# CDCgov/NowcastAutoGP

Measured on AMD Instinct MI355X. Metric: particle-logml/s (fit+forecast hot path: covariance assembly + Cholesky + logml + predictive per (particle, scenario) item), n=2048 64-particle SMC, higher is better.
Workload: dtype f64

## Files before the change

### nowcastautogp_amd/csrc/ngp_col_kernels.h

```cpp
#pragma once
#include <algorithm>

#include "ngp_mfma.h"

namespace ngp {

struct NoProbe {
    __device__ __forceinline__ void mark(int) {}
    template <class T>
    __device__ __forceinline__ void mark_after(int, T) {}
    __device__ __forceinline__ void drain() {}
    __device__ __forceinline__ void emit_diag(int, int, int) {}
    __device__ __forceinline__ void emit_col(int, int, int, int, int, int, bool) {}
    __device__ __forceinline__ void begin(int, int, int) {}
    __device__ __forceinline__ void sweep(int) {}
};

__device__ __forceinline__ void sqrt_and_rcp(double a, double &d, double &r) {
    double y = __builtin_amdgcn_rsq(a);
    const double h = 0.5 * a;
    y = y * fma(-h * y, y, 1.5);
    y = y * fma(-h * y, y, 1.5);
    d = a * y;
    d = fma(fma(-d, d, a), 0.5 * y, d);
    r = fma(fma(-d, y, 1.0), y, y);
}

__device__ __forceinline__ int tri(int r, int c) { return ((r * (r + 1)) >> 1) + c; }
constexpr int TRI = NB * (NB + 1) / 2;

template <class Probe = NoProbe>
__global__ __launch_bounds__(256, 4) void chol_diag_kernel(JobGeom g, ChunkPtrs p, int j, int k0) {
    __shared__ double Mt[TRI];
    __shared__ double Lt[TRI];
    __shared__ double pan[NB][4];
    __shared__ double dblk[16];
    __shared__ double dinvd[4];
    __shared__ double rdg[NB];
    __shared__ double logs[NB];
    __shared__ double Ts[TB][TB + 1];
    __shared__ int bad;
    const int item = blockIdx.x;
    const int tid = threadIdx.x, lane = tid & 63;
    const int wave = __builtin_amdgcn_readfirstlane(tid >> 6);
    const long ld = g.ld;
    double *Lit = p.L + (long)item * g.item_stride;
    double *Lj = Lit + (long)j * NB * ld;
    const int kmax = j * NB;
    const int r16 = lane & 15, q = lane >> 4;
    const int wr = wave >> 1, wc = wave & 1;
    Probe probe;
    probe.mark_after(0, lane);

    if (tid == 0) bad = 0;

    if (!(wr == 0 && wc == 1)) {
        double acc4[2][2][4];
#pragma unroll
        for (int a = 0; a < 2; ++a)
#pragma unroll
            for (int b = 0; b < 2; ++b)
#pragma unroll
                for (int r = 0; r < 4; ++r) acc4[a][b][r] = 0.0;
        const double *pa = Lj + (long)(32 * wr + r16) * ld + 2 * q;
        const double *pb = Lj + (long)(32 * wc + r16) * ld + 2 * q;
        double kt[2][2][4];
#pragma unroll
        for (int mt = 0; mt < 2; ++mt)
#pragma unroll
            for (int nt = 0; nt < 2; ++nt)
#pragma unroll
                for (int s = 0; s < 4; ++s)
                    kt[mt][nt][s] = Lj[(long)(32 * wr + 16 * mt + q + 4 * s) * ld + kmax +
                                       32 * wc + 16 * nt + r16];
        for (int kc = k0; kc < kmax; kc += 16) {
            double a[2][4], b[2][4];
#pragma unroll
            for (int u = 0; u < 2; ++u) {
                const f64x2 alo = *reinterpret_cast<const f64x2 *>(pa + (long)u * 16 * ld + kc);
                const f64x2 ahi = *reinterpret_cast<const f64x2 *>(pa + (long)u * 16 * ld + kc + 8);
                const f64x2 blo = *reinterpret_cast<const f64x2 *>(pb + (long)u * 16 * ld + kc);
                const f64x2 bhi = *reinterpret_cast<const f64x2 *>(pb + (long)u * 16 * ld + kc + 8);
                a[u][0] = alo.x; a[u][1] = alo.y; a[u][2] = ahi.x; a[u][3] = ahi.y;
                b[u][0] = blo.x; b[u][1] = blo.y; b[u][2] = bhi.x; b[u][3] = bhi.y;
            }
#pragma unroll
            for (int s = 0; s < 4; ++s)
#pragma unroll
                for (int nt = 0; nt < 2; ++nt) {
                    const Rot4 br = rot4(b[nt][s]);
#pragma unroll
                    for (int mt = 0; mt < 2; ++mt) mfma16_as_4(acc4[mt][nt], a[mt][s], br);
                }
        }
        f64x4 acc[2][2];
#pragma unroll
        for (int a = 0; a < 2; ++a)
#pragma unroll
            for (int b = 0; b < 2; ++b) acc[a][b] = to_d16(acc4[a][b]);
#pragma unroll
        for (int mt = 0; mt < 2; ++mt)
#pragma unroll
            for (int nt = 0; nt < 2; ++nt)
#pragma unroll
                for (int s = 0; s < 4; ++s) {
                    const int M = 32 * wr + 16 * mt + q + 4 * s, N = 32 * wc + 16 * nt + r16;
                    if (M >= N) Mt[tri(M, N)] = kt[mt][nt][s] - acc[mt][nt][s];
                }
    }
    __syncthreads();
    probe.mark_after(1, lane);

    const int bi = tid >> 4, bj = tid & 15;
    {
        double a[4][4];
#pragma unroll
        for (int r = 0; r < 4; ++r)
#pragma unroll
            for (int c = 0; c < 4; ++c) {
                const int R = 4 * bi + r, C = 4 * bj + c;
                a[r][c] = (R >= C) ? Mt[tri(R, C)] : 0.0;
            }
        for (int kb = 0; kb < NB / 4; ++kb) {
            if (bi == kb && bj == kb) {
                double dks[4];
#pragma unroll
                for (int kc = 0; kc < 4; ++kc) {
                    const double akk = a[kc][kc];
                    double dk, inv;
                    sqrt_and_rcp(akk, dk, inv);
                    if (!(akk > 0.0) && bad == 0) bad = 4 * kb + kc + 1;
                    dks[kc] = dk;
                    dinvd[kc] = inv;
                    rdg[4 * kb + kc] = inv;
#pragma unroll
                    for (int r = 0; r < 4; ++r)
                        if (r > kc) a[r][kc] *= inv;
#pragma unroll
                    for (int c = 0; c < 4; ++c)
                        if (c > kc) {
#pragma unroll
                            for (int r = 0; r < 4; ++r)
                                if (r >= c) a[r][c] -= a[r][kc] * a[c][kc];
                        }
                }
#pragma unroll
                for (int r = 0; r < 4; ++r)
#pragma unroll
                    for (int c = 0; c < 4; ++c) {
                        if (r == c) a[r][c] = dks[r];
                        if (c > r) a[r][c] = 0.0;
                        dblk[4 * r + c] = a[r][c];
                    }
            }
            __syncthreads();
            if (bj == kb && bi > kb) {
#pragma unroll
                for (int c = 0; c < 4; ++c) {
                    const double inv = dinvd[c];
#pragma unroll
                    for (int r = 0; r < 4; ++r) {
                        double v = a[r][c];
#pragma unroll
                        for (int pp = 0; pp < 4; ++pp)
                            if (pp < c) v -= a[r][pp] * dblk[4 * c + pp];
                        a[r][c] = v * inv;
                    }
                }
#pragma unroll
                for (int r = 0; r < 4; ++r)
#pragma unroll
                    for (int c = 0; c < 4; ++c) pan[4 * bi + r][c] = a[r][c];
            }
            __syncthreads();
            if (bj > kb && bi >= bj) {
                double li[4][4], lj[4][4];
#pragma unroll
                for (int r = 0; r < 4; ++r)
#pragma unroll
                    for (int pp = 0; pp < 4; ++pp) {
                        li[r][pp] = pan[4 * bi + r][pp];
                        lj[r][pp] = pan[4 * bj + r][pp];
                    }
#pragma unroll
                for (int pp = 0; pp < 4; ++pp)
#pragma unroll
                    for (int r = 0; r < 4; ++r)
#pragma unroll
                        for (int c = 0; c < 4; ++c) a[r][c] -= li[r][pp] * lj[c][pp];
            }
        }
#pragma unroll
        for (int r = 0; r < 4; ++r) {
            const int R = 4 * bi + r;
            f64x2 lo, hi;
            lo.x = (R >= 4 * bj) ? a[r][0] : 0.0;
            lo.y = (R >= 4 * bj + 1) ? a[r][1] : 0.0;
            hi.x = (R >= 4 * bj + 2) ? a[r][2] : 0.0;
            hi.y = (R >= 4 * bj + 3) ? a[r][3] : 0.0;
            double *dst = Lj + (long)R * ld + kmax + 4 * bj;
            *reinterpret_cast<f64x2 *>(dst) = lo;
            *reinterpret_cast<f64x2 *>(dst + 2) = hi;
#pragma unroll
            for (int c = 0; c < 4; ++c)
                if (R >= 4 * bj + c) Lt[tri(R, 4 * bj + c)] = a[r][c];
        }
    }
    __syncthreads();
    probe.mark_after(2, lane);
    if (tid < NB) logs[tid] = log(Lt[tri(tid, tid)]);

    if (tid < NB) {
        const int b = tid >> 4, c = tid & 15;
        double x[TB];
#pragma unroll
        for (int i = 0; i < TB; ++i) {
            double sum = (i == c) ? 1.0 : 0.0;
            int off = tri(TB * b + i, TB * b);
            if (i > 0) asm volatile("" : "+v"(off) : "v"(x[i - 1]));
            const double *lrow = &Lt[off];
#pragma unroll
            for (int pp = 0; pp < i; ++pp) sum -= lrow[pp] * x[pp];
            x[i] = sum * rdg[TB * b + i];
        }
#pragma unroll
        for (int i = 0; i < TB; ++i)
            if (i >= c) Mt[tri(TB * b + i, TB * b + c)] = x[i];
    }
    __syncthreads();
    probe.mark_after(3, lane);
    {
        const int ra = tid >> 4, cb = tid & 15;
        for (int dist = 1; dist < NB / TB; ++dist)
            for (int ct = dist; ct < NB / TB; ++ct) {
                const int jt = ct - dist;
                double t = 0.0;
                for (int kt = jt; kt < ct; ++kt)
#pragma unroll
                    for (int pp = 0; pp < TB; ++pp) {
                        const double mv = Mt[tri(TB * kt + pp, TB * jt + cb)];
                        t += Lt[tri(TB * ct + ra, TB * kt + pp)] * ((kt > jt || pp >= cb) ? mv : 0.0);
                    }
                Ts[ra][cb] = t;
                __syncthreads();
                double mv = 0.0;
#pragma unroll
                for (int pp = 0; pp < TB; ++pp) {
                    const double md = Mt[tri(TB * ct + ra, TB * ct + pp)];
                    mv -= ((pp <= ra) ? md : 0.0) * Ts[pp][cb];
                }
                Mt[tri(TB * ct + ra, TB * jt + cb)] = mv;
                __syncthreads();
            }
    }
    probe.mark_after(4, lane);
    {
        double *dv = p.dinv + (long)item * (NB * NB);
        for (int e = tid; e < NB * NB; e += 256) {
            const int strip = e >> 6, l = e & 63;
            const int cb4 = strip >> 2, jt = strip & 3;
            const int R = 4 * cb4 + (l & 3), C = 16 * jt + 4 * ((l >> 2) & 3) + (l >> 4);
            dv[e] = (R >= C) ? Mt[tri(R, C)] : 0.0;
        }
    }
    if (tid == 0) {
        double s = 0.0;
        for (int k = 0; k < NB; ++k) s += logs[k];
        p.logdet[item] += s;
        if (bad && p.info[item] == 0) p.info[item] = kmax + bad;
    }
    probe.mark_after(5, lane);
    probe.emit_diag(j, tid, item);
}

template <int NF>
struct Frag8 {
    f64x2 v[NF];
};
template <int NF>
__device__ __forceinline__ void load_frag8(Frag8<NF> &f, const double *p, long ld) {
#pragma unroll
    for (int u = 0; u < NF; ++u) f.v[u] = *reinterpret_cast<const f64x2 *>(p + (long)u * 16 * ld);
}
template <int NA>
__device__ __forceinline__ void mfma_frag8(double (&acc)[NA][4][4], const Frag8<NA> &a,
                                           const Frag8<4> &b) {
#pragma unroll
    for (int it = 0; it < 4; ++it) {
        const Rot4 br = rot4(b.v[it].x);
#pragma unroll
        for (int jt = 0; jt < NA; ++jt) mfma16_as_4(acc[jt][it], a.v[jt].x, br);
    }
#pragma unroll
    for (int it = 0; it < 4; ++it) {
        const Rot4 br = rot4(b.v[it].y);
#pragma unroll
        for (int jt = 0; jt < NA; ++jt) mfma16_as_4(acc[jt][it], a.v[jt].y, br);
    }
}

template <int NA>
__device__ __forceinline__ void gemm_rows(double (&acc)[NA][4][4], const double *pa,
                                          const double *pb, long ld, int k0, int k1) {
    if (k1 <= k0) return;
    Frag8<NA> a0, a1;
    Frag8<4> b0, b1;
    load_frag8(a0, pa + k0, ld);
    load_frag8(b0, pb + k0, ld);
    for (int kc = k0; kc < k1; kc += 16) {
        load_frag8(a1, pa + kc + 8, ld);
        load_frag8(b1, pb + kc + 8, ld);
        mfma_frag8(acc, a0, b0);
        if (kc + 16 < k1) {
            load_frag8(a0, pa + kc + 16, ld);
            load_frag8(b0, pb + kc + 16, ld);
        }
        mfma_frag8(acc, a1, b1);
    }
}

constexpr int EPI_PITCH = 66;
constexpr int EPI_M_BYTES = NB * NB * 8;
constexpr int EPI_WAVE_BYTES = 16 * EPI_PITCH * 8;
constexpr int EPI_LDS_BYTES = EPI_M_BYTES + 4 * EPI_WAVE_BYTES;

__device__ __forceinline__ void stage_mstrips(double *lds_m, const double *mstrips, int tid) {
#pragma unroll
    for (int i = 0; i < 8; ++i) {
        const int idx = tid + 256 * i;
        reinterpret_cast<f64x2 *>(lds_m)[idx] = reinterpret_cast<const f64x2 *>(mstrips)[idx];
    }
}

template <bool SHADOW = false, bool SYNTH = false, class Probe = NoProbe, bool KROWS = false>
__device__ __forceinline__ void solve_and_store_lds(const double (*acc4)[4][4], double *Lr,
                                                    const double *lds_m, long ld, int kmax,
                                                    int lane, double *buf, Probe &probe,
                                                    float *Lr32 = nullptr,
                                                    float *tmax_out = nullptr, int synth = 0,
                                                    const double *ksl = nullptr, int nit = 4) {
    double amax = 0.0;
    const int n16 = lane & 15, isub = lane >> 4;
    const int jj0 = 4 * (n16 >> 2) + isub;
    const double *ksl0 = ksl ? ksl + 15 - jj0 : nullptr;
    f64x2 kvr[8];
    double kvp[4][4];
    const int hrow = lane >> 5, c2 = 2 * (lane & 31);
    bool from_rows = KROWS && ksl0 == nullptr;
    if constexpr (SYNTH) from_rows = from_rows && synth == 0;
    auto k_elems = [&](int it, double (&kv)[4][4]) {
        if (ksl0) {
#pragma unroll
            for (int jt = 0; jt < 4; ++jt)
#pragma unroll
                for (int r = 0; r < 4; ++r)
                    kv[jt][r] = ksl0[((n16 + 4 * r) & 15) + 16 * (it - jt + 3)];
            return;
        }
        if constexpr (SYNTH) {
            if (synth) {
#pragma unroll
                for (int jt = 0; jt < 4; ++jt)
#pragma unroll
                    for (int r = 0; r < 4; ++r) {
                        const int i = 16 * it + ((n16 + 4 * r) & 15);
                        kv[jt][r] = (synth == 2 && i == 16 * jt + jj0) ? 1.0 : 0.0;
                    }
                return;
            }
        }
        if constexpr (!KROWS) {
#pragma unroll
            for (int jt = 0; jt < 4; ++jt)
#pragma unroll
                for (int r = 0; r < 4; ++r) {
                    const int i = 16 * it + ((n16 + 4 * r) & 15);
                    kv[jt][r] = Lr[(long)i * ld + kmax + 16 * jt + jj0];
                }
        }
    };
    auto load_k = [&](int it) {
        if constexpr (KROWS) {
            if (!from_rows) return;
#pragma unroll
            for (int i = 0; i < 8; ++i)
                kvr[i] = *reinterpret_cast<const f64x2 *>(Lr + (long)(16 * it + 2 * i + hrow) * ld + kmax + c2);
        } else {
            k_elems(it, kvp);
        }
    };
    auto take_k = [&](int it, double (&kv)[4][4]) {
        if constexpr (KROWS) {
            if (!from_rows) {
                k_elems(it, kv);
                return;
            }
#pragma unroll
            for (int i = 0; i < 8; ++i)
                *reinterpret_cast<f64x2 *>(buf + (2 * i + hrow) * EPI_PITCH + c2) = kvr[i];
#pragma unroll
            for (int jt = 0; jt < 4; ++jt)
#pragma unroll
                for (int r = 0; r < 4; ++r)
                    kv[jt][r] = buf[((n16 + 4 * r) & 15) * EPI_PITCH + 16 * jt + jj0];
        } else {
#pragma unroll
            for (int jt = 0; jt < 4; ++jt)
#pragma unroll
                for (int r = 0; r < 4; ++r) kv[jt][r] = kvp[jt][r];
        }
    };
    load_k(0);
#pragma unroll
    for (int it = 0; it < 4; ++it) {
        if (it >= nit) break;
        double c4[4][4];
        take_k(it, c4);
#pragma unroll
        for (int jt = 0; jt < 4; ++jt)
#pragma unroll
            for (int r = 0; r < 4; ++r) c4[jt][r] = c4[jt][r] - acc4[jt][it][r];
        probe.mark_after(12 + 3 * it, c4[3][3] + c4[0][0] + c4[1][2] + c4[2][1]);
        if (it + 1 < nit) load_k(it + 1);
        double ms[2][4];
        ms[0][0] = lds_m[lane];
#pragma unroll
        for (int cb4 = 0; cb4 < 16; ++cb4) {
            const int ct = cb4 >> 2;
            if (cb4 + 1 < 16) {
#pragma unroll
                for (int jt = 0; jt <= ((cb4 + 1) >> 2); ++jt)
                    ms[(cb4 + 1) & 1][jt] = lds_m[((cb4 + 1) * 4 + jt) * 64 + lane];
            }
            double R[4] = {0.0, 0.0, 0.0, 0.0};
#pragma unroll
            for (int jt = 0; jt <= ct; ++jt) {
#pragma unroll
                for (int r = 0; r < 4; ++r) R[r] = mfma4(ms[cb4 & 1][jt], c4[jt][r], R[r]);
            }
            double x = R[0];
            x += dpp_f64<ROW_ROR4, 0xF>(R[1], R[1]);
            x += dpp_f64<ROW_ROR8, 0xF>(R[2], R[2]);
            x += dpp_f64<ROW_ROR12, 0xF>(R[3], R[3]);
            buf[n16 * EPI_PITCH + 4 * cb4 + isub] = x;
        }
        probe.mark_after(13 + 3 * it, it);
#pragma unroll
        for (int w = 0; w < 8; ++w) {
            const int idx = w * 64 + lane, row = idx >> 5, cp = idx & 31;
            const f64x2 v = *reinterpret_cast<const f64x2 *>(buf + row * EPI_PITCH + 2 * cp);
            *reinterpret_cast<f64x2 *>(Lr + (long)(16 * it + row) * ld + kmax + 2 * cp) = v;
            if constexpr (SHADOW) {
                typedef float f32x2 __attribute__((ext_vector_type(2)));
                f32x2 vf;
                vf.x = (float)v.x;
                vf.y = (float)v.y;
                *reinterpret_cast<f32x2 *>(Lr32 + (long)(16 * it + row) * ld + kmax + 2 * cp) = vf;
                amax = fmax(amax, fmax(fabs(v.x), fabs(v.y)));
            }
        }
        probe.mark_after(14 + 3 * it, it);
        __builtin_amdgcn_sched_barrier(0);
    }
    if constexpr (SHADOW) {
#pragma unroll
        for (int off = 32; off > 0; off >>= 1) amax = fmax(amax, __shfl_xor(amax, off, 64));
        if (lane == 0) *tmax_out = __double2float_ru(amax);
    }
}

__device__ __forceinline__ void subtract_in_place_perm(double *rows, long ld, int c0,
                                                       const double (*acc4)[4][4], int lane,
                                                       bool fresh = false,
                                                       const double *ksl = nullptr, int nit = 4) {
    const int n16 = lane & 15, isub = lane >> 4;
    const int jj0 = 4 * (n16 >> 2) + isub;
    double *base = rows + c0 + jj0;
    long roff[4];
#pragma unroll
    for (int r = 0; r < 4; ++r) roff[r] = (long)((n16 + 4 * r) & 15) * ld;
    if (ksl) {
        const double *ksl0 = ksl + 15 - jj0;
#pragma unroll
        for (int it = 0; it < 4; ++it)
#pragma unroll
            for (int jt = 0; jt < 4; ++jt)
#pragma unroll
                for (int r = 0; r < 4; ++r)
                    base[(long)(16 * it) * ld + roff[r] + 16 * jt] =
                        ksl0[((n16 + 4 * r) & 15) + 16 * (it - jt + 3)] - acc4[jt][it][r];
        return;
    }
    if (fresh) {
#pragma unroll
        for (int it = 0; it < 4; ++it)
#pragma unroll
            for (int jt = 0; jt < 4; ++jt)
#pragma unroll
                for (int r = 0; r < 4; ++r)
                    base[(long)(16 * it) * ld + roff[r] + 16 * jt] = -acc4[jt][it][r];
        return;
    }
    double v[2][4][4];
#pragma unroll
    for (int jt = 0; jt < 4; ++jt)
#pragma unroll
        for (int r = 0; r < 4; ++r) v[0][jt][r] = base[roff[r] + 16 * jt];
#pragma unroll
    for (int it = 0; it < 4; ++it) {
        if (it >= nit) break;
        if (it + 1 < nit) {
#pragma unroll
            for (int jt = 0; jt < 4; ++jt)
#pragma unroll
                for (int r = 0; r < 4; ++r)
                    v[(it + 1) & 1][jt][r] = base[(long)(16 * (it + 1)) * ld + roff[r] + 16 * jt];
        }
#pragma unroll
        for (int jt = 0; jt < 4; ++jt)
#pragma unroll
            for (int r = 0; r < 4; ++r)
                base[(long)(16 * it) * ld + roff[r] + 16 * jt] = v[it & 1][jt][r] - acc4[jt][it][r];
    }
}

__device__ __forceinline__ void subtract_in_place_rows(double *rows, long ld, int c0,
                                                       const double (*acc4)[4][4], int lane,
                                                       double *tl, bool fresh = false,
                                                       const double *ksl = nullptr, int nit = 4) {
    const int n16 = lane & 15, isub = lane >> 4;
    const int jj0 = 4 * (n16 >> 2) + isub;
    const int hrow = lane >> 5, c2 = 2 * (lane & 31);
    double *base = rows + c0 + c2;
    auto load_rows = [&](int it, f64x2 (&kv)[8]) {
        if (ksl) {
#pragma unroll
            for (int i = 0; i < 8; ++i) {
                const int d = 63 + 16 * it + 2 * i + hrow - c2;
                kv[i].x = ksl[d];
                kv[i].y = ksl[d - 1];
            }
        } else if (fresh) {
#pragma unroll
            for (int i = 0; i < 8; ++i) kv[i].x = kv[i].y = 0.0;
        } else {
#pragma unroll
            for (int i = 0; i < 8; ++i)
                kv[i] = *reinterpret_cast<const f64x2 *>(base + (long)(16 * it + 2 * i + hrow) * ld);
        }
    };
    f64x2 kv[2][8];
    load_rows(0, kv[0]);
#pragma unroll
    for (int it = 0; it < 4; ++it) {
        if (it >= nit) break;
        if (it + 1 < nit) load_rows(it + 1, kv[(it + 1) & 1]);
#pragma unroll
        for (int jt = 0; jt < 4; ++jt)
#pragma unroll
            for (int r = 0; r < 4; ++r)
                tl[((n16 + 4 * r) & 15) * EPI_PITCH + 16 * jt + jj0] = acc4[jt][it][r];
#pragma unroll
        for (int i = 0; i < 8; ++i) {
            const f64x2 a = *reinterpret_cast<const f64x2 *>(tl + (2 * i + hrow) * EPI_PITCH + c2);
            f64x2 o;
            o.x = kv[it & 1][i].x - a.x;
            o.y = kv[it & 1][i].y - a.y;
            *reinterpret_cast<f64x2 *>(base + (long)(16 * it + 2 * i + hrow) * ld) = o;
        }
    }
}

__device__ __forceinline__ void struct_slice(double *ksl, const JobGeom &g, const ChunkPtrs &p,
                                             int item, int row0, int col0, int lane) {
    const double *tab = p.tab + (long)item * g.maxstat * g.R;
    const int d0 = row0 - col0 - 63;
    ksl[lane] = tab[(long)g.toep * (d0 + lane)];
    if (lane < 63) ksl[64 + lane] = tab[(long)g.toep * (d0 + 64 + lane)];
}
constexpr int TOEP_LDS_BYTES = 4 * 128 * 8;

struct ColStep {
    int j;
    int k0;
    int nmain;
    int ntiles;
    int groups;
    int splits;
    int first_touch;
    double c32, jitter;
};
__device__ __forceinline__ long tmax_index(const JobGeom &g, int row_tile, int col) {
    return (long)row_tile * g.nb0 + col;
}

template <bool MIXED, bool IDENT = false, bool TOEP = false>
__global__ __launch_bounds__(256, 2) void chol_col_kernel(JobGeom g, ChunkPtrs p, int Bc,
                                                          ColStep st) {
    __shared__ __attribute__((aligned(16))) char epi[EPI_LDS_BYTES + (TOEP ? TOEP_LDS_BYTES : 0)];
    const int wg = blockIdx.x;
    const int xcd = wg & 7, idx = wg >> 3;
    const int slot = (idx / st.groups) * 8 + xcd;
    const int grp = idx % st.groups;
    if (slot >= Bc) return;
    const int item = p.items ? p.items[slot] : slot;
    const int tid = threadIdx.x, lane = tid & 63;
    const int wave = __builtin_amdgcn_readfirstlane(tid >> 6);
    const int tile = grp * 4 + wave;
    bool valid = tile < st.ntiles;
    int kbeg = st.k0;
    int synth = 0;
    if constexpr (IDENT) {
        if (valid && tile >= st.nmain) {
            const int a = tile - st.nmain;
            if (a < g.nb0) {
                if (a > st.j) valid = false;
                else if (a * NB > kbeg) kbeg = a * NB;
                synth = (a == st.j) ? 2 : 1;
            }
        }
    }

    const int j = st.j;
    const long ld = g.ld;
    double *Lit = p.L + (long)item * g.item_stride;
    const int kmax = j * NB;
    const int r16 = lane & 15, q = lane >> 4;

    double acc4[4][4][4];
#pragma unroll
    for (int a = 0; a < 4; ++a)
#pragma unroll
        for (int b = 0; b < 4; ++b)
#pragma unroll
            for (int r = 0; r < 4; ++r) acc4[a][b][r] = 0.0;

    const int vt = valid ? tile : 0;
    const long rowbase = (vt < st.nmain) ? (long)(j + 1 + vt) * NB
                                         : (long)g.n0 + (long)(vt - st.nmain) * NB;
    double *Lr = Lit + rowbase * ld;
    const double *Lj = Lit + (long)j * NB * ld;
    const double *pa = Lj + (long)r16 * ld + 2 * q;
    const double *pb = Lr + (long)r16 * ld + 2 * q;
    if (valid) gemm_rows<4>(acc4, pa, pb, ld, kbeg, kmax);
    const double *ksl = nullptr;
    if constexpr (TOEP) {
        if (valid && tile < st.nmain && prog_structure(p.progs + item)) {
            double *sl = reinterpret_cast<double *>(epi + EPI_LDS_BYTES) + wave * 128;
            struct_slice(sl, g, p, item, (int)rowbase, kmax, lane);
            ksl = sl;
        }
    }
    stage_mstrips(reinterpret_cast<double *>(epi), p.dinv + (long)item * (NB * NB), tid);
    __syncthreads();
    if (!valid) return;
    NoProbe probe;
    if constexpr (MIXED) {
        const int rt = (tile < st.nmain) ? j + 1 + tile : g.nb0 + (tile - st.nmain);
        solve_and_store_lds<true>(
            acc4, Lr, reinterpret_cast<const double *>(epi), ld, kmax, lane,
            reinterpret_cast<double *>(epi + EPI_M_BYTES + wave * EPI_WAVE_BYTES), probe,
            p.L32 + (long)item * g.item_stride + rowbase * ld,
            p.tmax + (long)item * (g.nb0 + g.naux_pad / NB) * g.nb0 + tmax_index(g, rt, j));
    } else {
        solve_and_store_lds<false, IDENT>(
            acc4, Lr, reinterpret_cast<const double *>(epi), ld, kmax, lane,
            reinterpret_cast<double *>(epi + EPI_M_BYTES + wave * EPI_WAVE_BYTES), probe, nullptr,
            nullptr, synth, ksl);
    }
}

template <bool MIXED, class Probe = NoProbe, bool IDENT = false>
__global__ __launch_bounds__(256, 2) void chol_col_thin_kernel(JobGeom g, ChunkPtrs p, int Bc,
                                                               ColStep st) {
    constexpr int A_BYTES = NB * NB * 8;
    constexpr int TAIL = (4 * EPI_WAVE_BYTES > A_BYTES) ? 4 * EPI_WAVE_BYTES : A_BYTES;
    __shared__ __attribute__((aligned(1024))) char smem[EPI_M_BYTES + TAIL];
    typedef __attribute__((address_space(3))) void *lds_ptr;
    const int wg = blockIdx.x;
    const int xcd = wg & 7, idx = wg >> 3;
    const int slot = (idx / st.groups) * 8 + xcd;
    const int grp = idx % st.groups;
    if (slot >= Bc) return;
    const int item = p.items ? p.items[slot] : slot;
    const int tid = threadIdx.x, lane = tid & 63;
    const int wave = __builtin_amdgcn_readfirstlane(tid >> 6);
    const int tile = grp * 4 + wave;
    bool valid = tile < st.ntiles;
    const int j = st.j;
    const int kmax = j * NB, k0 = kmax - NB;
    bool update = true;
    int synth = 0;
    if constexpr (IDENT) {
        if (valid && tile >= st.nmain) {
            const int a = tile - st.nmain;
            if (a < g.nb0) {
                if (a > j) valid = false;
                else if (a * NB > k0) update = false;
                if (a == j) synth = 2;
            }
        }
    }
    const long ld = g.ld;
    double *Lit = p.L + (long)item * g.item_stride;
    const int r16 = lane & 15, q = lane >> 4;
    Probe probe;
    probe.mark_after(0, lane);

    {
        const __amdgpu_buffer_rsrc_t rl = __builtin_amdgcn_make_buffer_rsrc(
            Lit, 0, (int)(g.item_stride * (long)sizeof(double)), 0x00020000);
        const __amdgpu_buffer_rsrc_t rm = __builtin_amdgcn_make_buffer_rsrc(
            p.dinv + (long)item * (NB * NB), 0, NB * NB * 8, 0x00020000);
        const int rbit = lane >> 5, sl = lane & 31;
#pragma unroll
        for (int i = 0; i < 8; ++i) {
            const int key = (2 * i + rbit) & 7;
            const unsigned voff = (unsigned)((rbit * ld + 2 * (sl ^ key)) * 8);
            const unsigned soff = (unsigned)__builtin_amdgcn_readfirstlane(
                (int)((((long)kmax + 2 * (8 * wave + i)) * ld + k0) * 8));
            lds_ptr dst = (lds_ptr)(smem + EPI_M_BYTES + (8 * wave + i) * 1024);
            __builtin_amdgcn_raw_ptr_buffer_load_lds(rl, dst, 16, voff, soff, 0, 0);
        }
#pragma unroll
        for (int i = 0; i < 8; ++i) {
            lds_ptr dst = (lds_ptr)(smem + (8 * wave + i) * 1024);
            __builtin_amdgcn_raw_ptr_buffer_load_lds(rm, dst, 16, (unsigned)(lane * 16),
                                                     (unsigned)((8 * wave + i) * 1024), 0, 0);
        }
    }

    double acc4[4][4][4];
#pragma unroll
    for (int a = 0; a < 4; ++a)
#pragma unroll
        for (int b = 0; b < 4; ++b)
#pragma unroll
            for (int r = 0; r < 4; ++r) acc4[a][b][r] = 0.0;

    const int vt = valid ? tile : 0;
    const long rowbase = (vt < st.nmain) ? (long)(j + 1 + vt) * NB
                                         : (long)g.n0 + (long)(vt - st.nmain) * NB;
    double *Lr = Lit + rowbase * ld;
    const double *pb = Lr + (long)r16 * ld + k0 + 2 * q;
    const bool mult = valid && update;
    Frag8<4> b[4];
    if (mult) {
#pragma unroll
        for (int sg = 0; sg < 4; ++sg) load_frag8(b[sg], pb + 8 * sg, ld);
    }
    __syncthreads();
    probe.mark_after(1, lane);
    if (mult) {
        const char *Ab = smem + EPI_M_BYTES + r16 * 512;
        const int key = r16 & 7;
#pragma unroll
        for (int sg = 0; sg < 8; ++sg) {
            Frag8<4> a;
#pragma unroll
            for (int u = 0; u < 4; ++u)
                a.v[u] = *reinterpret_cast<const f64x2 *>(Ab + u * (16 * 512) +
                                                          (((4 * sg + q) ^ key) << 4));
            mfma_frag8(acc4, a, b[sg & 3]);
            if (sg + 4 < 8) load_frag8(b[sg & 3], pb + 8 * (sg + 4), ld);
        }
    }
    probe.mark_after(2, acc4[0][0][0] + acc4[3][3][3]);
    __syncthreads();
    probe.mark_after(3, lane);
    probe.mark_after(4, lane);
    if (!valid) return;
    double *buf = reinterpret_cast<double *>(smem + EPI_M_BYTES + wave * EPI_WAVE_BYTES);
    if constexpr (MIXED) {
        const int rt = (tile < st.nmain) ? j + 1 + tile : g.nb0 + (tile - st.nmain);
        solve_and_store_lds<true, false, Probe, true>(
            acc4, Lr, reinterpret_cast<const double *>(smem), ld, kmax, lane, buf, probe,
            p.L32 + (long)item * g.item_stride + rowbase * ld,
            p.tmax + (long)item * (g.nb0 + g.naux_pad / NB) * g.nb0 + tmax_index(g, rt, j));
    } else {
        int nit = (tile >= st.nmain && g.naux - NB * (tile - st.nmain) <= 16) ? 1 : 4;
        if (IDENT && tile < st.nmain && g.n_real - NB * (j + 1 + tile) <= 16) nit = 1;
        solve_and_store_lds<false, IDENT, Probe, true>(acc4, Lr, reinterpret_cast<const double *>(smem), ld,
                                          kmax, lane, buf, probe, nullptr, nullptr, synth, nullptr,
                                          nit);
    }
    probe.mark_after(5, lane);
    probe.drain();
    probe.mark_after(6, lane);
    probe.emit_col(j, lane, wg, wave, item, tile, true);
}

constexpr int LDS_KC = 16;

typedef float f32x4 __attribute__((ext_vector_type(4)));
typedef float f32x16 __attribute__((ext_vector_type(16)));


template <bool MIXED, class Probe = NoProbe, bool IDENT = false, int SPLITK = 0>
__global__ __launch_bounds__(256, 2) void chol_col_glds_kernel(JobGeom g, ChunkPtrs p, int Bc,
                                                               ColStep st) {
    constexpr int ROWB = 128, BLKB = 8 * ROWB + 128, STAGE = 32 * BLKB;
    auto row_off = [](int row) { return (row >> 3) * BLKB + (row & 7) * ROWB; };
    __shared__ __attribute__((aligned(1024))) char smem[2 * STAGE];
    typedef __attribute__((address_space(3))) void *lds_ptr;

    const int wg = blockIdx.x;
    const int xcd = wg & 7, idx = wg >> 3;
    const int per_item = SPLITK == 1 ? st.groups * st.splits : st.groups;
    const int slot = (idx / per_item) * 8 + xcd;
    const int grp = SPLITK == 1 ? (idx % per_item) / st.splits : idx % st.groups;
    const int piece = SPLITK == 1 ? (idx % per_item) % st.splits : 0;
    if (slot >= Bc) return;
    const int item = (MIXED && p.order) ? p.order[slot] : slot;
    const int tid = threadIdx.x, lane = tid & 63;
    const int wave = __builtin_amdgcn_readfirstlane(tid >> 6);
    const int ltile = wave >> 1, col = wave & 1;
    const int tile0 = grp * 2;
    const int tile = tile0 + ltile;
    bool valid = tile < st.ntiles;

    const int j = st.j;
    Probe probe;
    probe.mark(0);
    const long ld = g.ld;
    double *Lit = p.L + (long)item * g.item_stride;
    const int kmax = j * NB;
    bool structured = false;
    if constexpr (!MIXED && !IDENT) {
        if (g.toep && st.first_touch && valid && tile < st.nmain && !(col && tile == 0))
            structured = prog_structure(p.progs + item) != 0;
    }
    int kbeg = st.k0;
    int synth = 0;
    if constexpr (IDENT) {
        const int a = tile - st.nmain;
        if (tile < st.ntiles && a >= 0 && a < g.nb0) synth = (a == j) ? 2 : 1;
    }
    if (IDENT && tile0 >= st.nmain) {
        int kfirst = kmax + 1;
#pragma unroll
        for (int u = 0; u < 2; ++u) {
            const int a = tile0 + u - st.nmain;
            if (tile0 + u >= st.ntiles) continue;
            const int ks = (a >= g.nb0) ? st.k0 : (a > j) ? kmax + 1 : max(st.k0, a * NB);
            kfirst = min(kfirst, ks);
        }
        if (kfirst > kmax) return;
        kbeg = kfirst;
        const int a = tile - st.nmain;
        if (valid && a < g.nb0 && a > j) valid = false;
    }
    int nit = 4;
    if constexpr (!MIXED && SPLITK == 0) {
        if (IDENT && !valid) nit = 0;
        else if (valid && tile >= st.nmain && g.naux - NB * (tile - st.nmain) <= 16) nit = 1;
        else if (IDENT && valid && tile < st.nmain && g.n_real - NB * (j + 1 + tile) <= 16) nit = 1;
    }
    const int r16 = lane & 15, q = lane >> 4;
    auto tile_row0 = [&](int t) -> long {
        if (t >= st.ntiles) t = st.ntiles - 1;
        return (t < st.nmain) ? (long)(j + 1 + t) * NB : (long)g.n0 + (long)(t - st.nmain) * NB;
    };
    const __amdgpu_buffer_rsrc_t rsrc = __builtin_amdgcn_make_buffer_rsrc(
        Lit, 0, (int)(g.item_stride * (long)sizeof(double)), 0x00020000);
    long src_row0;
    if (wave < 2) src_row0 = (long)j * NB + 64 * wave;
    else src_row0 = tile_row0(tile0 + (wave - 2));
    const unsigned soff_base = (unsigned)__builtin_amdgcn_readfirstlane((int)(src_row0 * ld * 8));
    const unsigned row_step8 = (unsigned)(8 * ld * 8);
    const unsigned voff_even = (unsigned)(((lane >> 3) * ld + 2 * ((lane & 7) ^ ((lane >> 4) & 7))) * 8);
    const unsigned voff_odd = (unsigned)(((lane >> 3) * ld + 2 * ((lane & 7) ^ ((4 + (lane >> 4)) & 7))) * 8);
    auto stage = [&](int buf, int k) {
        const unsigned kb = (unsigned)k * 8u;
#pragma unroll
        for (int i = 0; i < 8; ++i) {
            lds_ptr dst = (lds_ptr)(smem + buf * STAGE + (8 * wave + i) * BLKB);
            __builtin_amdgcn_raw_ptr_buffer_load_lds(rsrc, dst, 16, (i & 1) ? voff_odd : voff_even,
                                                     soff_base + i * row_step8 + kb, 0, 0);
        }
    };
    unsigned a_addr[4], b_addr[4][4];
    {
        const int arow = 64 * col + r16;
        const int akey = (r16 >> 1) & 7;
#pragma unroll
        for (int s = 0; s < 4; ++s)
            a_addr[s] = (unsigned)(row_off(arow) + (((2 * s + (q >> 1)) ^ akey) << 4) + (q & 1) * 8);
#pragma unroll
        for (int r = 0; r < 4; ++r) {
            const int rr = (r16 + 4 * r) & 15;
            const int brow = 128 + 64 * ltile + rr;
            const int bkey = (rr >> 1) & 7;
#pragma unroll
            for (int s = 0; s < 4; ++s)
                b_addr[r][s] =
                    (unsigned)(row_off(brow) + (((2 * s + (q >> 1)) ^ bkey) << 4) + (q & 1) * 8);
        }
    }

    double acc4[4][4][4];
#pragma unroll
    for (int a = 0; a < 4; ++a)
#pragma unroll
        for (int b = 0; b < 4; ++b)
#pragma unroll
            for (int r = 0; r < 4; ++r) acc4[a][b][r] = 0.0;

    auto mult64 = [&](const char *buf, auto nit_c) {
        constexpr int NIT = decltype(nit_c)::value;
#pragma unroll
        for (int s = 0; s < 4; ++s) {
            double a[4];
#pragma unroll
            for (int u = 0; u < 4; ++u)
                a[u] = *reinterpret_cast<const double *>(buf + a_addr[s] + u * 2 * BLKB);
#pragma unroll
            for (int it = 0; it < NIT; ++it) {
                Rot4 br;
                br.r0 = *reinterpret_cast<const double *>(buf + b_addr[0][s] + it * 2 * BLKB);
                br.r1 = *reinterpret_cast<const double *>(buf + b_addr[1][s] + it * 2 * BLKB);
                br.r2 = *reinterpret_cast<const double *>(buf + b_addr[2][s] + it * 2 * BLKB);
                br.r3 = *reinterpret_cast<const double *>(buf + b_addr[3][s] + it * 2 * BLKB);
#pragma unroll
                for (int jt = 0; jt < 4; ++jt) mfma16_as_4(acc4[jt][it], a[jt], br);
            }
        }
    };

    if constexpr (SPLITK == 2) {
    } else if constexpr (!MIXED) {
        int nchunks = (kmax - kbeg) / LDS_KC;
        if constexpr (SPLITK == 1) {
            const int per = (nchunks + st.splits - 1) / st.splits;
            const int c0 = min(piece * per, nchunks);
            nchunks = min(c0 + per, nchunks) - c0;
            kbeg += c0 * LDS_KC;
        }
        if (nchunks > 0) {
            stage(0, kbeg);
            __syncthreads();
            if (IDENT && nit == 0) {
                for (int c = 0; c < nchunks; ++c) {
                    if (c + 1 < nchunks) stage((c & 1) ^ 1, kbeg + (c + 1) * LDS_KC);
                    __syncthreads();
                }
            } else if (nit == 1) {
                for (int c = 0; c < nchunks; ++c) {
                    const int cur = c & 1;
                    if (c + 1 < nchunks) stage(cur ^ 1, kbeg + (c + 1) * LDS_KC);
                    mult64(smem + cur * STAGE, std::integral_constant<int, 1>{});
                    __syncthreads();
                }
            } else {
                for (int c = 0; c < nchunks; ++c) {
                    const int cur = c & 1;
                    if (c + 1 < nchunks) stage(cur ^ 1, kbeg + (c + 1) * LDS_KC);
                    mult_chunk_pipelined<2 * BLKB>(acc4, smem + cur * STAGE, a_addr, b_addr);
                    __syncthreads();
                    if (c == 0) probe.mark(1);
                    if (c == nchunks / 2) probe.mark(2);
                }
            }
        }
    } else {
        const int nkt = j;
        const int nbt = g.nb0 + g.naux_pad / NB;
        const float *tm = p.tmax + (long)item * nbt * g.nb0;
        const int t1 = min(tile0 + 1, st.ntiles - 1);
        const int rt0 = (tile0 < st.nmain) ? j + 1 + tile0 : g.nb0 + (tile0 - st.nmain);
        const int rt1 = (t1 < st.nmain) ? j + 1 + t1 : g.nb0 + (t1 - st.nmain);
        const double lim = st.c32 * (p.progs[item].noise + st.jitter);
        unsigned long long m32lo, m32hi;
        {
            bool c[2];
#pragma unroll
            for (int h = 0; h < 2; ++h) {
                const int kt = lane + 64 * h;
                c[h] = false;
                if (kt < nkt) {
                    const float ta = fmaxf(tm[tmax_index(g, j, kt)], tm[tmax_index(g, j + 1, kt)]);
                    const float tb = fmaxf(tm[tmax_index(g, rt0, kt)], tm[tmax_index(g, rt1, kt)]);
                    c[h] = (double)ta * (double)tb <= lim;
                }
            }
            m32lo = __ballot(c[0]);
            m32hi = __ballot(c[1]);
        }
        const unsigned long long inlo = nkt >= 64 ? ~0ull : ((1ull << nkt) - 1ull);
        const unsigned long long inhi = nkt <= 64 ? 0ull : (nkt >= 128 ? ~0ull : ((1ull << (nkt - 64)) - 1ull));
        unsigned long long m64lo = inlo & ~m32lo, m64hi = inhi & ~m32hi;
        const int n32 = __popcll(m32lo) + __popcll(m32hi);
        const int n64 = __popcll(m64lo) + __popcll(m64hi);
        if (tid == 0 && p.mixcnt) {
            const unsigned nv = (unsigned)(2 * min(2, st.ntiles - tile0));
            atomicAdd(p.mixcnt + 2 * item, nv * (unsigned)n32);
            atomicAdd(p.mixcnt + 2 * item + 1, nv * (unsigned)n64);
        }
        auto pop = [](unsigned long long &lo, unsigned long long &hi) -> int {
            if (lo) {
                const int b = __builtin_ctzll(lo);
                lo &= lo - 1;
                return b;
            }
            const int b = __builtin_ctzll(hi);
            hi &= hi - 1;
            return 64 + b;
        };

        if (n32 > 0) {
            const __amdgpu_buffer_rsrc_t rsrc32 = __builtin_amdgcn_make_buffer_rsrc(
                p.L32 + (long)item * g.item_stride, 0, (int)(g.item_stride * (long)sizeof(float)),
                0x00020000);
            const unsigned soff32 = (unsigned)__builtin_amdgcn_readfirstlane((int)(src_row0 * ld * 4));
            const unsigned row_step32 = (unsigned)(8 * ld * 4);
            const unsigned v32_even = (unsigned)((lane >> 3) * ld * 4 + 16 * ((lane & 7) ^ ((lane >> 4) & 7)));
            const unsigned v32_odd = (unsigned)((lane >> 3) * ld * 4 + 16 * ((lane & 7) ^ ((4 + (lane >> 4)) & 7)));
            auto stage32 = [&](int buf, int k) {
                const unsigned kb = (unsigned)k * 4u;
#pragma unroll
                for (int i = 0; i < 8; ++i) {
                    lds_ptr dst = (lds_ptr)(smem + buf * STAGE + (8 * wave + i) * BLKB);
                    __builtin_amdgcn_raw_ptr_buffer_load_lds(rsrc32, dst, 16,
                                                             (i & 1) ? v32_odd : v32_even,
                                                             soff32 + i * row_step32 + kb, 0, 0);
                }
            };
            const int r32 = lane & 31, h = lane >> 5;
            unsigned a32[2][4], b32[2][4];
#pragma unroll
            for (int blk = 0; blk < 2; ++blk) {
                const int arow = 64 * col + 32 * blk + r32;
                const int brow = 128 + 64 * ltile + 32 * blk + r32;
#pragma unroll
                for (int u = 0; u < 4; ++u) {
                    a32[blk][u] = (unsigned)(row_off(arow) + (((2 * u + h) ^ ((arow >> 1) & 7)) << 4));
                    b32[blk][u] = (unsigned)(row_off(brow) + (((2 * u + h) ^ ((brow >> 1) & 7)) << 4));
                }
            }
            f32x16 acc32[2][2];
            double acc64p[2][2][16];
#pragma unroll
            for (int a = 0; a < 2; ++a)
#pragma unroll
                for (int b = 0; b < 2; ++b)
#pragma unroll
                    for (int v = 0; v < 16; ++v) {
                        acc32[a][b][v] = 0.f;
                        acc64p[a][b][v] = 0.0;
                    }
            unsigned long long lo = m32lo, hi = m32hi;
            const int nch = 2 * n32;
            int kt_cur = pop(lo, hi), sub = 1;
            stage32(0, kt_cur * NB);
            __syncthreads();
            for (int c = 0; c < nch; ++c) {
                const int cur = c & 1;
                if (c + 1 < nch) {
                    if (sub == 2) {
                        kt_cur = pop(lo, hi);
                        sub = 0;
                    }
                    stage32(cur ^ 1, kt_cur * NB + 32 * sub);
                    ++sub;
                }
                const char *buf = smem + cur * STAGE;
#pragma unroll
                for (int u = 0; u < 4; ++u) {
                    f32x4 av[2], bv[2];
#pragma unroll
                    for (int blk = 0; blk < 2; ++blk) {
                        av[blk] = *reinterpret_cast<const f32x4 *>(buf + a32[blk][u]);
                        bv[blk] = *reinterpret_cast<const f32x4 *>(buf + b32[blk][u]);
                    }
#pragma unroll
                    for (int e = 0; e < 4; ++e)
#pragma unroll
                        for (int a = 0; a < 2; ++a)
#pragma unroll
                            for (int b = 0; b < 2; ++b)
                                acc32[a][b] = __builtin_amdgcn_mfma_f32_32x32x2f32(
                                    av[a][e], bv[b][e], acc32[a][b], 0, 0, 0);
                }
                if (c & 1) {
#pragma unroll
                    for (int a = 0; a < 2; ++a)
#pragma unroll
                        for (int b = 0; b < 2; ++b)
#pragma unroll
                            for (int v = 0; v < 16; ++v) {
                                acc64p[a][b][v] += (double)acc32[a][b][v];
                                acc32[a][b][v] = 0.f;
                            }
                }
                __syncthreads();
            }
            constexpr int P64 = 65;
            double *t64 = reinterpret_cast<double *>(smem) + wave * (32 * P64);
            static_assert(4 * 32 * P64 * 8 <= 2 * STAGE, "hand-over tiles must fit the stage buffers");
            const int jj0 = 4 * (r16 >> 2) + q;
#pragma unroll
            for (int a = 0; a < 2; ++a) {
#pragma unroll
                for (int b = 0; b < 2; ++b)
#pragma unroll
                    for (int v = 0; v < 16; ++v)
                        t64[((v & 3) + 8 * (v >> 2) + 4 * h) * P64 + 32 * b + r32] = acc64p[a][b][v];
                __syncthreads();
#pragma unroll
                for (int jl = 0; jl < 2; ++jl)
#pragma unroll
                    for (int it = 0; it < 4; ++it)
#pragma unroll
                        for (int r = 0; r < 4; ++r)
                            acc4[2 * a + jl][it][r] =
                                t64[(16 * jl + jj0) * P64 + 16 * it + ((r16 + 4 * r) & 15)];
                __syncthreads();
            }
        }
        if (n64 > 0) {
            unsigned long long lo = m64lo, hi = m64hi;
            const int nch = 4 * n64;
            int kt_cur = pop(lo, hi), sub = 1;
            stage(0, kt_cur * NB);
            __syncthreads();
            for (int c = 0; c < nch; ++c) {
                const int cur = c & 1;
                if (c + 1 < nch) {
                    if (sub == 4) {
                        kt_cur = pop(lo, hi);
                        sub = 0;
                    }
                    stage(cur ^ 1, kt_cur * NB + LDS_KC * sub);
                    ++sub;
                }
                mult_chunk_pipelined<2 * BLKB>(acc4, smem + cur * STAGE, a_addr, b_addr);
                __syncthreads();
            }
        }
    }
    if constexpr (SPLITK == 1) {
        double *mine = p.splitk_part +
                       ((((long)slot * SPLITK_SLOTS + (long)grp * st.splits + piece) * 4 + wave) *
                        (64 * 64)) + lane;
#pragma unroll
        for (int jt = 0; jt < 4; ++jt)
#pragma unroll
            for (int it = 0; it < 4; ++it)
#pragma unroll
                for (int r = 0; r < 4; ++r) mine[((jt * 4 + it) * 4 + r) * 64] = acc4[jt][it][r];
        return;
    }
    if constexpr (SPLITK == 2) {
        const double *part = p.splitk_part +
                             ((((long)slot * SPLITK_SLOTS + (long)grp * st.splits) * 4 + wave) *
                              (64 * 64)) + lane;
#pragma unroll
        for (int jt = 0; jt < 4; ++jt)
#pragma unroll
            for (int it = 0; it < 4; ++it)
#pragma unroll
                for (int r = 0; r < 4; ++r) acc4[jt][it][r] = part[((jt * 4 + it) * 4 + r) * 64];
        for (int q2 = 1; q2 < st.splits; ++q2) {
            const double *pq = part + (long)q2 * 4 * (64 * 64);
            double v[4][4][4];
#pragma unroll
            for (int jt = 0; jt < 4; ++jt)
#pragma unroll
                for (int it = 0; it < 4; ++it)
#pragma unroll
                    for (int r = 0; r < 4; ++r) v[jt][it][r] = pq[((jt * 4 + it) * 4 + r) * 64];
#pragma unroll
            for (int jt = 0; jt < 4; ++jt)
#pragma unroll
                for (int it = 0; it < 4; ++it)
#pragma unroll
                    for (int r = 0; r < 4; ++r) acc4[jt][it][r] += v[jt][it][r];
        }
    }
    static_assert(EPI_LDS_BYTES + TOEP_LDS_BYTES <= 2 * STAGE,
                  "epilogue LDS must fit the stage buffers");
    probe.mark(3);
    const double *ksl = nullptr;
    if (structured) {
        double *sl = reinterpret_cast<double *>(smem + EPI_LDS_BYTES) + wave * 128;
        struct_slice(sl, g, p, item, (int)tile_row0(tile), col ? kmax + NB : kmax, lane);
        ksl = sl;
    }
    stage_mstrips(reinterpret_cast<double *>(smem), p.dinv + (long)item * (NB * NB), tid);
    __syncthreads();
    probe.mark(4);
    if (!valid) return;

    double *Lr = Lit + tile_row0(tile) * ld;
    if (col) {
        subtract_in_place_rows(Lr, ld, (j + 1) * NB, acc4, lane,
                               reinterpret_cast<double *>(smem + EPI_M_BYTES + wave * EPI_WAVE_BYTES),
                               IDENT && synth != 0, ksl, nit);
    } else if constexpr (MIXED) {
        const int rt = (tile < st.nmain) ? j + 1 + tile : g.nb0 + (tile - st.nmain);
        solve_and_store_lds<true>(
            acc4, Lr, reinterpret_cast<const double *>(smem), ld, kmax, lane,
            reinterpret_cast<double *>(smem + EPI_M_BYTES + wave * EPI_WAVE_BYTES), probe,
            p.L32 + (long)item * g.item_stride + tile_row0(tile) * ld,
            p.tmax + (long)item * (g.nb0 + g.naux_pad / NB) * g.nb0 + tmax_index(g, rt, j));
    } else {
        solve_and_store_lds<false, IDENT>(
            acc4, Lr, reinterpret_cast<const double *>(smem), ld, kmax, lane,
            reinterpret_cast<double *>(smem + EPI_M_BYTES + wave * EPI_WAVE_BYTES), probe, nullptr,
            nullptr, synth, ksl, nit);
    }
    probe.mark(5);
    probe.drain();
    probe.mark(6);
    probe.emit_col(j, lane, wg, wave, item, tile, false);
}

template <class Probe>
void launch_chol_diag_t(const JobGeom &g, const ChunkPtrs &p, int Bc, int j, int k0, hipStream_t s) {
    hipLaunchKernelGGL(chol_diag_kernel<Probe>, dim3(Bc), dim3(256), 0, s, g, p, j, k0);
}

template <class Probe>
void launch_chol_col_t(const JobGeom &g, const ChunkPtrs &p, int Bc, int j, int mode, int k0,
                     hipStream_t s, const DevSpec *sp) {
    ColStep st{};
    const bool mixed = p.L32 != nullptr && sp != nullptr;
    if (mixed) {
        st.c32 = sp->mixed_tau / (64.0 * 5.9604644775390625e-08);
        st.jitter = sp->jitter;
    }
    st.j = j;
    st.k0 = k0;
    st.nmain = (mode == COL_AUX) ? 0 : g.nb0 - 1 - j;
    st.ntiles = st.nmain + g.naux_pad / NB;
    if (st.ntiles <= 0) return;
    const int bpad = (Bc + 7) / 8 * 8;
    const dim3 blk(256);
    st.first_touch = (mode == COL_FAT || (mode == COL_FULL && k0 == 0 && j == 0)) ? 1 : 0;
    if (mode == COL_FAT) {
        st.groups = (st.ntiles + 1) / 2;
        const dim3 grid(st.groups * bpad);
        int splits = 1;
        if (!mixed && !g.aux_identity && p.splitk_part) {
            const int nchunks = j * NB / LDS_KC;
            splits = std::min(std::min(8, SPLITK_SLOTS / std::max(st.groups, 1)),
                              std::min(nchunks / 8, 384 / std::max(st.groups * Bc, 1)));
        }
        st.splits = std::max(splits, 1);
        if (splits >= 2) {
            hipLaunchKernelGGL((chol_col_glds_kernel<false, Probe, false, 1>),
                               dim3(st.groups * splits * bpad), blk, 0, s, g, p, Bc, st);
            hipLaunchKernelGGL((chol_col_glds_kernel<false, Probe, false, 2>), grid, blk, 0, s, g, p,
                               Bc, st);
        } else if (mixed)
            hipLaunchKernelGGL((chol_col_glds_kernel<true, Probe>), grid, blk, 0, s, g, p, Bc, st);
        else if (g.aux_identity)
            hipLaunchKernelGGL((chol_col_glds_kernel<false, Probe, true>), grid, blk, 0, s, g, p, Bc, st);
        else
            hipLaunchKernelGGL((chol_col_glds_kernel<false, Probe>), grid, blk, 0, s, g, p, Bc, st);
    } else if (mode == COL_THIN && k0 == j * NB - NB && j > 0) {
        st.groups = (st.ntiles + 3) / 4;
        const dim3 grid(st.groups * bpad);
        if (mixed)
            hipLaunchKernelGGL((chol_col_thin_kernel<true, Probe>), grid, blk, 0, s, g, p, Bc, st);
        else if (g.aux_identity)
            hipLaunchKernelGGL((chol_col_thin_kernel<false, Probe, true>), grid, blk, 0, s, g, p, Bc, st);
        else
            hipLaunchKernelGGL((chol_col_thin_kernel<false, Probe>), grid, blk, 0, s, g, p, Bc, st);
    } else {
        st.groups = (st.ntiles + 3) / 4;
        const dim3 grid(st.groups * bpad);
        if (mixed)
            hipLaunchKernelGGL(chol_col_kernel<true>, grid, blk, 0, s, g, p, Bc, st);
        else if (g.aux_identity)
            hipLaunchKernelGGL((chol_col_kernel<false, true>), grid, blk, 0, s, g, p, Bc, st);
        else if (g.toep && st.first_touch)
            hipLaunchKernelGGL((chol_col_kernel<false, false, true>), grid, blk, 0, s, g, p, Bc, st);
        else
            hipLaunchKernelGGL(chol_col_kernel<false>, grid, blk, 0, s, g, p, Bc, st);
    }
}

}
```

Measured before the change: 17160.

## Share triangular-solve work between paired waves and pack M-strips in LDS

For the non-mixed, non-identity, non-split-K column kernel, the wave that solves a tile now handles only the first three 16-row sub-blocks. It hands the last sub-block's accumulators through LDS to its partner wave, which runs the remaining solve step after its in-place subtraction. This balances epilogue work between the solve wave and the subtract wave. The diagonal inverse strips are staged in a packed lower-triangular layout to free LDS room for the hand-off buffer and shared Toeplitz slices. The cost is extra LDS traffic, more complex indexing and a longer critical path on the subtract wave.

```diff
diff --git a/nowcastautogp_amd/csrc/ngp_col_kernels.h b/nowcastautogp_amd/csrc/ngp_col_kernels.h
--- a/nowcastautogp_amd/csrc/ngp_col_kernels.h
+++ b/nowcastautogp_amd/csrc/ngp_col_kernels.h
@@ -324,15 +324,36 @@
 constexpr int EPI_WAVE_BYTES = 16 * EPI_PITCH * 8;
 constexpr int EPI_LDS_BYTES = EPI_M_BYTES + 4 * EPI_WAVE_BYTES;
 
+constexpr int EPI_MP_BYTES = 40 * 64 * 8;
+template <bool PACKED>
+__device__ __forceinline__ constexpr int mstrip(int cb4, int jt) {
+    return PACKED ? 2 * (cb4 >> 2) * ((cb4 >> 2) + 1) + (cb4 & 3) * ((cb4 >> 2) + 1) + jt : 4 * cb4 + jt;
+}
+
+template <bool PACKED = false>
 __device__ __forceinline__ void stage_mstrips(double *lds_m, const double *mstrips, int tid) {
-#pragma unroll
-    for (int i = 0; i < 8; ++i) {
-        const int idx = tid + 256 * i;
-        reinterpret_cast<f64x2 *>(lds_m)[idx] = reinterpret_cast<const f64x2 *>(mstrips)[idx];
-    }
-}
-
-template <bool SHADOW = false, bool SYNTH = false, class Probe = NoProbe, bool KROWS = false>
+    if constexpr (PACKED) {
+#pragma unroll
+        for (int i = 0; i < 5; ++i) {
+            const int idx = tid + 256 * i;
+            const int ps = idx >> 5;
+            const int ct = (ps >= 4) + (ps >= 12) + (ps >= 24);
+            const int rem = ps - 2 * ct * (ct + 1);
+            const int cq = rem / (ct + 1), jt = rem - cq * (ct + 1);
+            reinterpret_cast<f64x2 *>(lds_m)[idx] =
+                reinterpret_cast<const f64x2 *>(mstrips)[(4 * (4 * ct + cq) + jt) * 32 + (idx & 31)];
+        }
+    } else {
+#pragma unroll
+        for (int i = 0; i < 8; ++i) {
+            const int idx = tid + 256 * i;
+            reinterpret_cast<f64x2 *>(lds_m)[idx] = reinterpret_cast<const f64x2 *>(mstrips)[idx];
+        }
+    }
+}
+
+template <bool SHADOW = false, bool SYNTH = false, class Probe = NoProbe, bool KROWS = false,
+          bool PACKED = false, int IT0 = 0>
 __device__ __forceinline__ void solve_and_store_lds(const double (*acc4)[4][4], double *Lr,
                                                     const double *lds_m, long ld, int kmax,
                                                     int lane, double *buf, Probe &probe,
@@ -410,9 +431,9 @@
                 for (int r = 0; r < 4; ++r) kv[jt][r] = kvp[jt][r];
         }
     };
-    load_k(0);
-#pragma unroll
-    for (int it = 0; it < 4; ++it) {
+    load_k(IT0);
+#pragma unroll
+    for (int it = IT0; it < 4; ++it) {
         if (it >= nit) break;
         double c4[4][4];
         take_k(it, c4);
@@ -423,14 +444,14 @@
         probe.mark_after(12 + 3 * it, c4[3][3] + c4[0][0] + c4[1][2] + c4[2][1]);
         if (it + 1 < nit) load_k(it + 1);
         double ms[2][4];
-        ms[0][0] = lds_m[lane];
+        ms[0][0] = lds_m[mstrip<PACKED>(0, 0) * 64 + lane];
 #pragma unroll
         for (int cb4 = 0; cb4 < 16; ++cb4) {
             const int ct = cb4 >> 2;
             if (cb4 + 1 < 16) {
 #pragma unroll
                 for (int jt = 0; jt <= ((cb4 + 1) >> 2); ++jt)
-                    ms[(cb4 + 1) & 1][jt] = lds_m[((cb4 + 1) * 4 + jt) * 64 + lane];
+                    ms[(cb4 + 1) & 1][jt] = lds_m[mstrip<PACKED>(cb4 + 1, jt) * 64 + lane];
             }
             double R[4] = {0.0, 0.0, 0.0, 0.0};
 #pragma unroll
@@ -572,11 +593,12 @@
 }
 
 __device__ __forceinline__ void struct_slice(double *ksl, const JobGeom &g, const ChunkPtrs &p,
-                                             int item, int row0, int col0, int lane) {
+                                             int item, int row0, int col0, int lane,
+                                             int nent = 127) {
     const double *tab = p.tab + (long)item * g.maxstat * g.R;
     const int d0 = row0 - col0 - 63;
     ksl[lane] = tab[(long)g.toep * (d0 + lane)];
-    if (lane < 63) ksl[64 + lane] = tab[(long)g.toep * (d0 + 64 + lane)];
+    if (lane < nent - 64) ksl[64 + lane] = tab[(long)g.toep * (d0 + 64 + lane)];
 }
 constexpr int TOEP_LDS_BYTES = 4 * 128 * 8;
 
@@ -825,10 +847,11 @@
     const long ld = g.ld;
     double *Lit = p.L + (long)item * g.item_stride;
     const int kmax = j * NB;
-    bool structured = false;
+    bool structured = false, structured_j = false;
     if constexpr (!MIXED && !IDENT) {
-        if (g.toep && st.first_touch && valid && tile < st.nmain && !(col && tile == 0))
-            structured = prog_structure(p.progs + item) != 0;
+        if (g.toep && st.first_touch && valid && tile < st.nmain)
+            structured_j = prog_structure(p.progs + item) != 0;
+        structured = structured_j && !(col && tile == 0);
     }
     int kbeg = st.k0;
     int synth = 0;
@@ -1177,37 +1200,76 @@
                     for (int r = 0; r < 4; ++r) acc4[jt][it][r] += v[jt][it][r];
         }
     }
-    static_assert(EPI_LDS_BYTES + TOEP_LDS_BYTES <= 2 * STAGE,
+    constexpr bool SHARE = !MIXED && !IDENT && SPLITK == 0;
+    constexpr int M_BYTES = SHARE ? EPI_MP_BYTES : EPI_M_BYTES;
+    constexpr int HAND_OFF = M_BYTES + 4 * EPI_WAVE_BYTES;
+    constexpr int HAND_BYTES = 16 * 64 * 8;
+    constexpr int PAIR_SLICE = 192;
+    constexpr int TOEP_OFF = SHARE ? HAND_OFF + 2 * HAND_BYTES : EPI_LDS_BYTES;
+    static_assert(TOEP_OFF + (SHARE ? 2 * PAIR_SLICE * 8 : TOEP_LDS_BYTES) <= 2 * STAGE,
                   "epilogue LDS must fit the stage buffers");
     probe.mark(3);
-    const double *ksl = nullptr;
-    if (structured) {
-        double *sl = reinterpret_cast<double *>(smem + EPI_LDS_BYTES) + wave * 128;
+    const bool share = SHARE && valid && nit == 4 && j > 0;
+    f64x2 *hand = reinterpret_cast<f64x2 *>(smem + HAND_OFF) + ltile * (8 * 64);
+    if (share && !col) {
+#pragma unroll
+        for (int jt = 0; jt < 4; ++jt)
+#pragma unroll
+            for (int h = 0; h < 2; ++h) {
+                f64x2 v;
+                v.x = acc4[jt][3][2 * h];
+                v.y = acc4[jt][3][2 * h + 1];
+                hand[(2 * jt + h) * 64 + lane] = v;
+            }
+    }
+    const double *ksl = nullptr, *ksl_j = nullptr;
+    if constexpr (SHARE) {
+        double *ps = reinterpret_cast<double *>(smem + TOEP_OFF) + ltile * PAIR_SLICE;
+        if (structured) {
+            if (col) struct_slice(ps, g, p, item, (int)tile_row0(tile), kmax + NB, lane, 64);
+            else struct_slice(ps + 64, g, p, item, (int)tile_row0(tile), kmax, lane);
+            ksl = col ? ps : ps + 64;
+        }
+        if (structured_j) ksl_j = ps + 64;
+    } else if (structured) {
+        double *sl = reinterpret_cast<double *>(smem + TOEP_OFF) + wave * 128;
         struct_slice(sl, g, p, item, (int)tile_row0(tile), col ? kmax + NB : kmax, lane);
         ksl = sl;
     }
-    stage_mstrips(reinterpret_cast<double *>(smem), p.dinv + (long)item * (NB * NB), tid);
+    stage_mstrips<SHARE>(reinterpret_cast<double *>(smem), p.dinv + (long)item * (NB * NB), tid);
     __syncthreads();
     probe.mark(4);
     if (!valid) return;
 
     double *Lr = Lit + tile_row0(tile) * ld;
+    const double *lds_m = reinterpret_cast<const double *>(smem);
+    double *tl = reinterpret_cast<double *>(smem + M_BYTES + wave * EPI_WAVE_BYTES);
     if (col) {
-        subtract_in_place_rows(Lr, ld, (j + 1) * NB, acc4, lane,
-                               reinterpret_cast<double *>(smem + EPI_M_BYTES + wave * EPI_WAVE_BYTES),
-                               IDENT && synth != 0, ksl, nit);
+        subtract_in_place_rows(Lr, ld, (j + 1) * NB, acc4, lane, tl, IDENT && synth != 0, ksl, nit);
+        if constexpr (SHARE) {
+            if (share) {
+#pragma unroll
+                for (int jt = 0; jt < 4; ++jt)
+#pragma unroll
+                    for (int h = 0; h < 2; ++h) {
+                        const f64x2 v = hand[(2 * jt + h) * 64 + lane];
+                        acc4[jt][3][2 * h] = v.x;
+                        acc4[jt][3][2 * h + 1] = v.y;
+                    }
+                solve_and_store_lds<false, false, Probe, false, true, 3>(
+                    acc4, Lr, lds_m, ld, kmax, lane, tl, probe, nullptr, nullptr, 0, ksl_j, 4);
+            }
+        }
     } else if constexpr (MIXED) {
         const int rt = (tile < st.nmain) ? j + 1 + tile : g.nb0 + (tile - st.nmain);
         solve_and_store_lds<true>(
-            acc4, Lr, reinterpret_cast<const double *>(smem), ld, kmax, lane,
-            reinterpret_cast<double *>(smem + EPI_M_BYTES + wave * EPI_WAVE_BYTES), probe,
+            acc4, Lr, lds_m, ld, kmax, lane, tl, probe,
             p.L32 + (long)item * g.item_stride + tile_row0(tile) * ld,
             p.tmax + (long)item * (g.nb0 + g.naux_pad / NB) * g.nb0 + tmax_index(g, rt, j));
     } else {
-        solve_and_store_lds<false, IDENT>(
-            acc4, Lr, reinterpret_cast<const double *>(smem), ld, kmax, lane,
-            reinterpret_cast<double *>(smem + EPI_M_BYTES + wave * EPI_WAVE_BYTES), probe, nullptr,
-            nullptr, synth, ksl, nit);
+        solve_and_store_lds<false, IDENT, Probe, false, SHARE>(
+            acc4, Lr, lds_m, ld, kmax, lane, tl, probe, nullptr, nullptr, synth, ksl,
+            share ? 3 : nit);
     }
     probe.mark(5);
     probe.drain();
```

Result: faster. 17360 (median of 6 runs) (+1.1%).
